# giesselmann/STRique

Hardware: AMD Instinct MI355X
Metric: reads/s for STRique 'count' on 50 kb r9.4 signals (higher is better)
Workload: dtype f32

## Files before the change

strique_amd/csrc/screen_kernels.h:

```cpp
#pragma once
#include <hip/hip_runtime.h>
#include <stdint.h>
#include "align_kernels.h"

#define STRQ_SCREEN_R 14
#define STRQ_SCREEN_S 6
#define STRQ_SCREEN_SEG 4
#define STRQ_SCREEN_CHUNK_COLS 128
#define STRQ_SCREEN_MAX_WINDOWS 4
#define STRQ_SCREEN2_CPL 5
#define STRQ_SCREEN2_LPF 29
#define STRQ_SCREEN2_LANE_B 32

namespace strq {

struct ScreenParams {
    int32_t sc;
    int32_t hh, v;
    int32_t cadd;
    int32_t slack;
    int32_t merge_gap;
    int32_t max_cand;
    int32_t margin;
};
// ... 4 lines not shown
    const int32_t* band_lo;
    int32_t* out;
    int32_t tsize;
    int32_t n, m, k, col_off;
    int32_t n_chunks;
    int32_t lane_last;
};

struct Screen2Task {
    const uint8_t* levels;
    const float* table[2];
    const int32_t* band_lo[2];
    int32_t* out[2];
    int32_t tsize[2], k[2];
    int32_t n, col_off, n_chunks;
};

struct ScreenWindows {
    int32_t n_win;
    int32_t lo[STRQ_SCREEN_MAX_WINDOWS], hi[STRQ_SCREEN_MAX_WINDOWS];
    float lower_bound;
    float upper_bound;
    int32_t n_cand;
};

int screen_plan(const AlignParams& p, int samples, int max_n, ScreenParams* sp);
static inline bool screen_flank_ok(int m) { return m >= 2 * STRQ_SCREEN_R && m <= 64 * STRQ_SCREEN_R; }
size_t screen_lds_bytes(int tsize);
int launch_screen(hipStream_t stream, const ScreenTask* tasks, int n_groups, int* queue, const ScreenParams& sp,
                  size_t lds_bytes, int tables_per_cu, int n_cu);
int screen2_plan(const AlignParams& p, int samples, int max_n, int merge, ScreenParams* sp);
static inline bool screen2_flank_ok(int m, int k) { return k >= 1 && k <= STRQ_SCREEN2_LPF * STRQ_SCREEN2_CPL && m == k * STRQ_SCREEN_S; }
size_t screen2_lds_bytes(int tsize_a, int tsize_b);
int launch_screen2(hipStream_t stream, const Screen2Task* tasks, int n_groups, int* queue, const ScreenParams& sp,
                   size_t lds_bytes, int groups_per_cu, int n_cu, int merge);
int launch_screen_windows(hipStream_t stream, const ScreenTask* tasks, int n_groups, const ScreenParams& sp,
                          const int32_t* bound_scaled, ScreenWindows* out, const int32_t* list = nullptr, const int32_t* theta_list = nullptr);

}
```

strique_amd/csrc/screen_kernels.hip:

```cpp
#include "strq_opt.h"
#include <hip/hip_runtime.h>
#include <stdint.h>
#include <stdlib.h>
#include <cmath>
#include "screen_kernels.h"

namespace strq {

namespace {

constexpr int R = STRQ_SCREEN_R, S = STRQ_SCREEN_S, SEG = STRQ_SCREEN_SEG;
constexpr int G = 2, C = 3;
static_assert(R == 14 && S == 6, "class expansion below is written for 14 rows per lane, 6 samples per class");

__device__ __forceinline__ int dpp_shr1(int v, int fill)
{
    return __builtin_amdgcn_update_dpp(fill, v, 0x138, 0xF, 0xF, false);
}
__device__ __forceinline__ int dpp_shr1_open(int v)
{
    return __builtin_amdgcn_mov_dpp(v, 0x138, 0xF, 0xF, true);
}
__device__ __forceinline__ int med3i(int a, int lo, int hi)
{
    int r;
    asm("v_med3_i32 %0, %1, %2, %3" : "=v"(r) : "v"(a), "v"(lo), "v"(hi));
    return r;
}
#define STRQ_SCREEN_BIAS 0x00800000
#ifndef STRQ_SCREEN_WPE
#define STRQ_SCREEN_WPE 6
#endif
__device__ __forceinline__ int max3i(int a, int b, int c)
{
    int r;
    asm("v_max3_f32 %0, %1, %2, %3" : "=v"(r) : "v"(a), "v"(b), "v"(c));
    return r;
}
// ... 239 lines not shown
            if (act) {
#pragma unroll
                for (int r = RPC * c; r < RPC * c + RPC; ++r) {
                    const int diagA = r == 0 ? upS : T[r - 1];
                    const int ta = max3i(diagA + scA[c], T[r], ta_prev);
                    if (r > 0) {
                        const int tb = max3i(ta_prev2 + scB[(r - 1) / RPC], ta_prev, tb_prev2);
                        T[r - 1] = tb; tb_prev2 = tb;
                    }
                    ta_prev2 = ta_prev; ta_prev = ta;
                }
                if (c == CPL - 1) {
                    const int tb = max3i(ta_prev2 + scB[c], ta_prev, tb_prev2);
                    T[R2 - 1] = tb;
                    SbotA = ta_prev;
                    upS = upB;
                    if constexpr (GROUPED) {
                        if (glast) { const int d = tb - gpot; gmax = d > gmax ? d : gmax; }
                    } else {
                        const int cA = ta_prev - potA + STRQ_SCREEN_BIAS, cB = okB ? tb - potBn + STRQ_SCREEN_BIAS : cA;
                        cmax = max3i(cmax, cA, cB);
                    }
                }
            }
            scA[c] = score(qa, c);
            if (c > 0) scB[c - 1] = score(qb, c - 1);
            if (c == CPL - 1) scB[c] = score(qb, c);
        }
        potB = potBn;
        qq = qn;
    }
};

__device__ __forceinline__ int load_chunk2(const Screen2Task& tk, int chunk, int lane)
{
    const int idx = (chunk * 64 + lane) * 2;
    int a = 0, b = 0;
    if (idx < tk.n) a = tk.levels[idx];
    if (idx + 1 < tk.n) b = tk.levels[idx + 1];
    return (a * 2) | ((b * 2) << 16);
}

template <int RPC, int CMG>
__device__ __forceinline__ void screen2_body(const Screen2Task* __restrict__ tasks, int n_groups, int* __restrict__ queue, const ScreenParams& sp)
{
    constexpr int R2 = RPC * CPL, MERGE = S / RPC;
    extern __shared__ uint32_t lds_all[];
    __shared__ int next_group;
    const int lane = threadIdx.x & 63, wave = threadIdx.x >> 6;
    const char* ldsb = reinterpret_cast<const char*>(lds_all);
    for (;;) {
        __syncthreads();
        if (threadIdx.x == 0) next_group = atomicAdd(queue, 1);
        __syncthreads();
        const int gi = __builtin_amdgcn_readfirstlane(next_group);
        if (gi >= n_groups) break;
        const Screen2Task& t0 = tasks[(size_t)gi * SEG];
        int base[2], zero_idx[2];
        base[0] = 0; zero_idx[0] = (t0.tsize[0] + 1) & ~1;
        base[1] = zero_idx[0] + 2; zero_idx[1] = base[1] + ((t0.tsize[1] + 1) & ~1);
        {
            uint16_t* dst = reinterpret_cast<uint16_t*>(lds_all);
            const float scf = (float)sp.sc;
#pragma unroll
            for (int f = 0; f < 2; ++f) {
                for (int i = threadIdx.x; i < t0.tsize[f]; i += 64 * SEG) dst[base[f] + i] = (uint16_t)(MERGE * ((int)ceilf(t0.table[f][i] * scf) + sp.cadd));
                if (threadIdx.x == 0) { dst[zero_idx[f]] = 0; dst[zero_idx[f] + 1] = 0; }
            }
        }
        __syncthreads();
        const Screen2Task& tk = tasks[(size_t)gi * SEG + wave];
        if (tk.n <= 0) continue;

        Lane2Const lc;
        const int f = lane >= LB ? 1 : 0, lf = lane - f * LB;
        {
#pragma unroll
            for (int c = 0; c < CPL; ++c) {
                const int k = lf * CPL + c;
                if (lf < LPF && k < tk.k[f]) {
                    const uint32_t d = (uint32_t)tk.band_lo[f][k];
                    const int lo = (int)(d & 255u), w1 = (int)((d >> 8) & 255u), off = (int)(d >> 16);
                    lc.lo2[c] = lo * 2; lc.hi2[c] = (lo + w1) * 2;
                    lc.off[c] = (base[f] + off - lo) * 2;
                } else {
                    lc.lo2[c] = 0; lc.hi2[c] = 0; lc.off[c] = zero_idx[f] * 2;
                }
            }
        }
        const uint64_t top_mask = 1ull | (1ull << LB);
        const int lMa = (tk.k[0] - 1) / CPL, lMb = LB + (tk.k[1] - 1) / CPL;
        Screen2<RPC, CMG> s2{ldsb, lc, top_mask, lane, tk.n, sp.hh};
        {
#pragma unroll
            for (int r = 0; r < R2; ++r) s2.T[r] = STRQ_SCREEN_BIAS;
            s2.SbotA = STRQ_SCREEN_BIAS; s2.upS = STRQ_SCREEN_BIAS;
            s2.potB = STRQ_SCREEN_BIAS - 2 * lane * sp.hh;
            s2.cmax = STRQ_SCREEN_BIAS; s2.gpot = 0; s2.gmax = 0;
        }
        const int nsteps = (tk.n + 1) / 2 + 63;
        int qcur = load_chunk2(tk, 0, lane);
        s2.prime(qcur);
        for (int t0s = 0; t0s < nsteps; t0s += 64) {
            const int qnext = load_chunk2(tk, t0s / 64 + 1, lane);
            const bool full = (t0s >= 63) && (2 * (t0s + 64) <= tk.n);
            const int send = nsteps - t0s < 64 ? nsteps - t0s : 64;
            if (full) {
                constexpr int U = CMG > 2 ? CMG : 2;
                s2.gmax = 0;
#pragma unroll 1
                for (int s = 0; s < 64 - U; s += U) {
#pragma unroll
                    for (int u = 0; u < U; ++u) s2.template step<false>(0, qcur, s + u + 1, u % CMG == 0, u % CMG == CMG - 1);
                }
#pragma unroll
                for (int u = 0; u < U - 1; ++u) s2.template step<false>(0, qcur, 64 - U + u + 1, u % CMG == 0, u % CMG == CMG - 1);
                s2.template step<false>(0, qnext, 0, CMG == 1, true);
                if constexpr (CMG > 1) s2.cmax = s2.gmax + STRQ_SCREEN_BIAS;
            } else {
                for (int s = 0; s < send; ++s) {
                    const int qsrc = s == 63 ? qnext : qcur, snext = (s + 1) & 63;
                    s2.template step<true>(t0s + s + 1, qsrc, snext);
                }
            }
            const int cma = __builtin_amdgcn_readlane(s2.cmax, lMa) - STRQ_SCREEN_BIAS;
            const int cmb = __builtin_amdgcn_readlane(s2.cmax, lMb) - STRQ_SCREEN_BIAS;
            if (lane == 0) { tk.out[0][t0s / 64] = cma; tk.out[1][t0s / 64] = cmb; }
            s2.cmax = STRQ_SCREEN_BIAS;
            qcur = qnext;
        }
    }
}

}

size_t screen2_lds_bytes(int tsize_a, int tsize_b)
{
    return (size_t)(((tsize_a + 1) & ~1) + 2 + ((tsize_b + 1) & ~1) + 2) * 2;
}

#ifndef STRQ_SCREEN3_CMG
#define STRQ_SCREEN3_CMG 2
#endif
#define STRQ_SCREEN2_ATTR(WPE_) __attribute__((amdgpu_flat_work_group_size(64 * STRQ_SCREEN_SEG, 64 * STRQ_SCREEN_SEG), amdgpu_waves_per_eu(WPE_, WPE_)))
__global__ void STRQ_SCREEN2_ATTR(6) align_screen3_kernel(const Screen2Task* __restrict__ tasks, int n_groups, int* __restrict__ queue, ScreenParams sp) { screen2_body<2, STRQ_SCREEN3_CMG>(tasks, n_groups, queue, sp); }
__global__ void STRQ_SCREEN2_ATTR(4) align_screen1_kernel(const Screen2Task* __restrict__ tasks, int n_groups, int* __restrict__ queue, ScreenParams sp) { screen2_body<6, 1>(tasks, n_groups, queue, sp); }

__global__ void __launch_bounds__(256)
screen_windows_kernel(const ScreenTask* __restrict__ tasks, int n_groups, ScreenParams sp,
                      const int32_t* __restrict__ bound_scaled, ScreenWindows* __restrict__ out,
                      const int32_t* __restrict__ list, const int32_t* __restrict__ theta_list)
{
    const int lane = threadIdx.x & 63;
    const int idx = blockIdx.x * (blockDim.x >> 6) + (threadIdx.x >> 6);
    if (idx >= n_groups) return;
    const int g = list ? list[idx] : idx;
    const ScreenTask* tg = tasks + (size_t)g * SEG;
    const int m = tg[0].m, lM = tg[0].lane_last;
    const int shift = -m * sp.v;
    int vmax = 0;
    for (int w = 0; w < SEG; ++w) {
        if (tg[w].n <= 0) continue;
        for (int c = lane; c < tg[w].n_chunks; c += 64) { const int v = tg[w].out[c]; vmax = v > vmax ? v : vmax; }
    }
#pragma unroll
    for (int d = 32; d >= 1; d >>= 1) { const int o = __shfl_xor(vmax, d, 64); vmax = o > vmax ? o : vmax; }
    ScreenWindows r;
    r.n_win = 0; r.n_cand = 0;
    for (int k = 0; k < STRQ_SCREEN_MAX_WINDOWS; ++k) { r.lo[k] = 0; r.hi[k] = 0; }
    const int drop = (sp.margin > 0 ? sp.margin : m) + 2 * sp.slack;
    int theta = theta_list ? theta_list[idx] : vmax - drop;
    if (!theta_list && sp.max_cand > 0) {
        auto count_at = [&](int t) {
            int n = 0;
            for (int w = 0; w < SEG; ++w) {
                if (tg[w].n <= 0) continue;
                for (int c = lane; c < tg[w].n_chunks; c += 64) n += tg[w].out[c] >= t;
            }
#pragma unroll
// ... 96 lines not shown
        if (hh < 1 || smax + v + hh > 65000.0) continue;
        const double top = 64.0 * R * (smax + v) + ((double)max_n + 256.0) * hh + smax + v + hh + (double)STRQ_SCREEN_BIAS;
        if (top > 2.0e9) continue;
        sp->sc = sc; sp->hh = (int)hh; sp->v = (int)v; sp->cadd = (int)(hh + v);
        {
            const double rows = 64.0 * R, maxval = rows * (double)p.dist_offset;
            double p2 = 1.0; while (p2 < maxval) p2 *= 2.0;
            const double adds = rows * (1.0 + (double)p.dist_offset / -(double)p.ext_h);
            const double e = adds * p2 / 16777216.0;
            if (!(e < 1.0e4)) continue;
            sp->slack = ((int)std::ceil(e) + 1) * sc;
        }
        sp->merge_gap = 3072; sp->margin = 0; sp->max_cand = 0;
        return 1;
    }
    return 0;
}

int screen2_plan(const AlignParams& p, int samples, int max_n, int merge, ScreenParams* sp)
{
    if (merge != 1 && merge != 3) return 0;
    if (!screen_plan(p, samples, max_n, sp)) return 0;
    while (sp->sc >= 16) {
        const double smax = std::ceil((double)p.dist_offset * sp->sc);
        if ((double)merge * (smax + sp->cadd) <= 65000.0) return 1;
        if ((sp->hh & 1) || (sp->v & 1)) return 0;
        sp->slack = (sp->slack / sp->sc) * (sp->sc / 2);
        sp->sc /= 2; sp->hh /= 2; sp->v /= 2; sp->cadd = sp->hh + sp->v;
    }
    return 0;
}

int launch_screen2(hipStream_t stream, const Screen2Task* tasks, int n_groups, int* queue, const ScreenParams& sp,
                   size_t lds_bytes, int groups_per_cu, int n_cu, int merge)
{
    if (n_groups <= 0) return 0;
    if (merge != 3 && merge != 1) return 2;
    auto kern = merge == 3 ? align_screen3_kernel : align_screen1_kernel;
    if (merge == 1 && groups_per_cu > 4) groups_per_cu = 4;
    if (groups_per_cu > 6) groups_per_cu = 6;
    (void)hipFuncSetAttribute((const void*)kern, hipFuncAttributeMaxDynamicSharedMemorySize, (int)lds_bytes);
    hipLaunchKernelGGL(kern, dim3(groups_per_cu * n_cu), dim3(64 * SEG), lds_bytes, stream, tasks, n_groups, queue, sp);
    return hipGetLastError() == hipSuccess ? 0 : 1;
}

int launch_screen(hipStream_t stream, const ScreenTask* tasks, int n_groups, int* queue, const ScreenParams& sp,
                  size_t lds_bytes, int tables_per_cu, int n_cu)
{
    if (n_groups <= 0) return 0;
    (void)hipFuncSetAttribute((const void*)align_screen_kernel, hipFuncAttributeMaxDynamicSharedMemorySize, (int)lds_bytes);
    hipLaunchKernelGGL(align_screen_kernel, dim3(tables_per_cu * n_cu), dim3(64 * SEG), lds_bytes, stream, tasks, n_groups, queue, sp);
    return hipGetLastError() == hipSuccess ? 0 : 1;
}

int launch_screen_windows(hipStream_t stream, const ScreenTask* tasks, int n_groups, const ScreenParams& sp,
                          const int32_t* bound_scaled, ScreenWindows* out, const int32_t* list, const int32_t* theta_list)
{
    if (n_groups <= 0) return 0;
    hipLaunchKernelGGL(screen_windows_kernel, dim3((n_groups + 3) / 4), dim3(256), 0, stream, tasks, n_groups, sp, bound_scaled, out, list, theta_list);
    return hipGetLastError() == hipSuccess ? 0 : 1;
}

}
```

strique_amd/csrc/strq_align_api.hip:

```cpp
#include <hip/hip_runtime.h>
#include <algorithm>
#include <cmath>
#include <climits>
#include <cstring>
#include <cstdlib>
#include <time.h>
#include <unistd.h>
#include <map>
#include <mutex>
#include <string>
#include <tuple>
#include <numeric>
#include <vector>
#include "../../include/strique_hip.h"
#include "strq_ctx.h"
#include "align_kernels.h"
#include "lut_kernels.h"
#include "align_generic.h"

using namespace strq;

#define STRQ_DBG(...) do { if (strq::opt("STRQ_DEBUG")) { fprintf(stderr, "[strq] " __VA_ARGS__); fprintf(stderr, "\n"); fflush(stderr); } } while (0)

namespace strq {
// ... 259 lines not shown
    if (hard_count > hard_cap) { c->err = "too many borderline table entries"; return STRQ_ERR_DEVICE; }
    bool any_rebuild = false;
    for (int j = 0; j < nj; ++j) any_rebuild |= info[j].n_hard < 0;
    auto level_vals_of = [&](int read, float* dst) -> int {
        STRQ_HIP(c, hipMemcpy(dst, b.d_level_val + (size_t)read * 256, 256 * 4, hipMemcpyDeviceToHost));
        return STRQ_OK;
    };
    if (hard_count > 0) {
        std::vector<HardEntry> he(hard_count); std::vector<float> hv(hard_count);
        STRQ_HIP(c, hipMemcpy(he.data(), d_hard, (size_t)hard_count * sizeof(HardEntry), hipMemcpyDeviceToHost));
        float lv[256]; int last_read = -1;
        for (int i = 0; i < hard_count; ++i) {
            const int rd = b.job_read[he[i].job];
            if (rd != last_read) { const int rc = level_vals_of(rd, lv); if (rc) return rc; last_read = rd; }
            hv[i] = host_cell_score(c->ap, lv[he[i].level], b.job_cls[he[i].job][he[i].k]);
        }
        STRQ_HIP(c, hipMemcpyAsync(d_hard_vals, hv.data(), (size_t)hard_count * 4, hipMemcpyHostToDevice, st));
        if (launch_lut_patch(st, d_jobs, d_hard, d_hard_vals, hard_count)) { c->err = "patch launch failed"; return STRQ_ERR_DEVICE; }
        STRQ_HIP(c, hipStreamSynchronize(st));
        if (b.handed) *b.handed = he;
    } else if (b.handed) b.handed->clear();
    if (any_rebuild) for (int j = 0; j < nj; ++j) if (info[j].n_hard < 0) {
        const int kk = jobs[j].k;
        std::vector<float> tab((size_t)kk * 256); std::vector<int32_t> blo(kk);
        float lv[256];
        { const int rc = level_vals_of(b.job_read[j], lv); if (rc) return rc; }
        for (int x = 0; x < kk; ++x) {
            float* row = &tab[(size_t)x * 256];
            for (int q = 0; q < 256; ++q) row[q] = host_cell_score(c->ap, lv[q], b.job_cls[j][x]);
            blo[x] = (int32_t)((255u << 8) | ((uint32_t)(x * 256) << 16));
        }
        STRQ_HIP(c, hipMemcpy(jobs[j].table, tab.data(), tab.size() * 4, hipMemcpyHostToDevice));
        STRQ_HIP(c, hipMemcpy(jobs[j].band_lo, blo.data(), (size_t)kk * 4, hipMemcpyHostToDevice));
        info[j].total = kk * 256;
    }
    b.hard_count = hard_count;
    return STRQ_OK;
}

static uint8_t* table3_slot(strq_ctx* c, size_t tab_off, int j)
{
    const size_t o = tab_off * 3 + (size_t)j * 8;
    return c->tables3.as<uint8_t>() + o - o % 4;
}

static int build_tables(CorePlan& p)
{
    strq_ctx* c = p.c; const AlignCoreIn& in = p.in;
    const int nb = p.nb, nj = p.nj;
    std::vector<LutJob>& jobs = p.jobs;
    jobs.resize(nj);
    TableBuild b;
    b.nj = nj; b.max_k = p.max_k; b.jobs = &jobs; b.d_level_val = in.d_level_val; b.after_tables = in.after_tables; b.info = &p.info;
    b.job_read.resize(nj); b.job_cls.resize(nj);
    for (int j = 0; j < nj; ++j) {
        const int i = p.job_align[j];
        jobs[j].level_val = in.d_level_val + (size_t)in.read[i] * 256;
        jobs[j].cls_val = c->flank_cls.as<float>() + p.cls_off[i] + p.job_k0[j];
        jobs[j].table = c->tables.as<float>() + p.tab_off[j];
        jobs[j].table3 = table3_slot(c, p.tab_off[j], j);
        jobs[j].band_lo = c->band_lo.as<int32_t>() + p.desc_off[j];
        jobs[j].k = p.job_k[j]; jobs[j].pad_ = 0;
        b.job_read[j] = in.read[i];
        b.job_cls[j] = &p.h_cls[p.cls_off[i] + p.job_k0[j]];
    }
    const int rc = run_table_build(c, p.st, b);
    if (rc) return rc;
    p.tab_total.assign(nb, 0);
    for (int j = 0; j < nj; ++j) p.tab_total[p.job_align[j]] = std::max(p.tab_total[p.job_align[j]], p.info[j].total);
    p.out.n_hard = b.hard_count;
    return STRQ_OK;
}

static void read_switches(CorePlan& p)
{
    const strq_ctx* c = p.c;
    p.collapsed = p.S == 6 && c->ap.open_h == c->ap.ext_h && c->ap.open_v == c->ap.ext_v;
    if (const char* e = strq::opt("STRQ_SEG")) { const int v = atoi(e); if (v >= 1 && v <= 4) p.seg_want = v; }
    if (const char* e = strq::opt("STRQ_TABLES")) { const int v = atoi(e); if (v >= 1 && v <= 8) p.max_tables = v; }
    if (const char* e = strq::opt("STRQ_MAX_WAVES")) { const int v = atoi(e); if (v >= 4 && v <= 16) p.max_waves = v; }
    p.allow_pack = p.collapsed && !strq::opt("STRQ_NO_PACK");
    if (const char* e = strq::opt("STRQ_OVERLAP")) { const int v = atoi(e); p.ov_cap = v > 0 ? v : (1 << 30); p.ov_fixed = true; }
    p.scr_forced = strq::opt("STRQ_SCREEN_ALWAYS") != nullptr;
    const char* mode_opt = strq::opt("STRQ_SCREEN_MODE");
    p.mode_fine = mode_opt && std::strcmp(mode_opt, "fine") == 0;
    p.mode_coarse = mode_opt && std::strcmp(mode_opt, "coarse") == 0;
}


struct ScreenJob {
    int flanks = 1;
    std::vector<int> al;
    std::vector<ScreenTask> views;
    std::vector<Screen2Task> t2;
    std::vector<int32_t> bound;
    std::vector<size_t> out_off;
    size_t out_words = 0, lds_bytes = 0;
    double steps = 0;
};

struct ScreenRules {
    int merge;
    int groups_per_cu;
    const char* lds_err;
    bool below_bound_free;
    bool count_untaken;
    bool judge;
    double max_cols;
    int* pause; int* fail;
};

static void screen_tasks(CorePlan& p, const ScreenParams& sp, ScreenJob& j)
{
    constexpr int SSEG = STRQ_SCREEN_SEG;
    const AlignCoreIn& in = p.in;
    const int F = j.flanks, ng = (int)j.al.size() / F;
    if (F == 2) j.t2.resize((size_t)ng * SSEG);
    j.views.resize(j.al.size() * SSEG);
    j.bound.resize(j.al.size());
    j.out_off.assign(j.al.size() * SSEG, 0);
    for (int g = 0; g < ng; ++g) {
        const int* a = &j.al[(size_t)g * F];
        const int n = in.n[a[0]];
        const int m_big = F == 2 ? std::max(in.m[a[0]], in.m[a[1]]) : in.m[a[0]];
        const int ov_worst = align_segment_overlap(p.c->ap, m_big), ov_s = overlap_for(p, m_big, ov_worst, 16);
        Piece pc[SSEG];
        const int used = cut(n, SSEG, ov_s, pc);
        j.lds_bytes = std::max(j.lds_bytes, F == 2 ? screen2_lds_bytes(p.info[p.J0[a[0]]].total, p.info[p.J0[a[1]]].total) : screen_lds_bytes(p.info[p.J0[a[0]]].total));
        for (int f = 0; f < F; ++f)
            j.bound[(size_t)g * F + f] = used <= 1 ? INT32_MIN / 2 : (ov_s >= ov_worst ? 0 : (int32_t)std::ceil((double)align_segment_min_score(p.c->ap, in.m[a[f]], ov_s) * sp.sc));
        for (int w = 0; w < SSEG; ++w) {
            Screen2Task t; std::memset(&t, 0, sizeof(t));
            t.levels = in.d_levels + in.read_off[in.read[a[0]]] + pc[w].col_off;
            t.n = pc[w].n; t.col_off = pc[w].col_off;
            t.n_chunks = pc[w].n > 0 ? (align_num_steps(pc[w].n) + 63) / 64 : 0;
            for (int f = 0; f < F; ++f) {
                const LutJob& job = p.jobs[p.J0[a[f]]];
                t.table[f] = job.table; t.band_lo[f] = job.band_lo; t.tsize[f] = p.info[p.J0[a[f]]].total; t.k[f] = in.k[a[f]];
                ScreenTask v; std::memset(&v, 0, sizeof(v));
                v.n = pc[w].n; v.m = in.m[a[f]]; v.k = in.k[a[f]]; v.col_off = pc[w].col_off; v.n_chunks = t.n_chunks;
                if (F == 2) v.lane_last = f * STRQ_SCREEN2_LANE_B + (in.k[a[f]] - 1) / STRQ_SCREEN2_CPL;
                else { v.levels = t.levels; v.table = t.table[0]; v.band_lo = t.band_lo[0]; v.tsize = t.tsize[0]; v.lane_last = (v.m - 1) / STRQ_SCREEN_R; }
                j.out_off[((size_t)g * F + f) * SSEG + w] = j.out_words; j.out_words += (size_t)t.n_chunks;
                j.views[((size_t)g * F + f) * SSEG + w] = v;
            }
            if (pc[w].n > 0) j.steps += align_num_steps(pc[w].n);
            if (F == 2) j.t2[(size_t)g * SSEG + w] = t;
        }
    }
}

static int run_screen(CorePlan& p, ScreenJob& j, const ScreenParams& sp, const ScreenRules& r)
{
    constexpr int SSEG = STRQ_SCREEN_SEG;
    strq_ctx* c = p.c; const AlignCoreIn& in = p.in;
    hipStream_t st = p.st;
    const int nv = (int)j.al.size();
    if (j.lds_bytes > 160 * 1024 - 64) { c->err = r.lds_err; return STRQ_ERR_UNSUPPORTED; }
    const int groups = std::max(1, std::min(r.groups_per_cu, (int)((160 * 1024 - 64) / j.lds_bytes)));
    auto aligned = [](size_t bytes) { return (bytes + 255) & ~(size_t)255; };
    const size_t t2_bytes = aligned(j.t2.size() * sizeof(Screen2Task)), task_bytes = aligned(j.views.size() * sizeof(ScreenTask));
    const size_t bound_bytes = aligned((size_t)nv * 4), win_bytes = aligned((size_t)nv * sizeof(ScreenWindows));
    STRQ_HIP(c, c->screen.reserve(t2_bytes + task_bytes + bound_bytes + win_bytes + j.out_words * 4 + 256));
    char* base = c->screen.as<char>();
    Screen2Task* d_t2 = reinterpret_cast<Screen2Task*>(base);
    ScreenTask* d_st = reinterpret_cast<ScreenTask*>(base + t2_bytes);
    int32_t* d_bound = reinterpret_cast<int32_t*>(base + t2_bytes + task_bytes);
    ScreenWindows* d_win = reinterpret_cast<ScreenWindows*>(base + t2_bytes + task_bytes + bound_bytes);
    int32_t* d_out = reinterpret_cast<int32_t*>(base + t2_bytes + task_bytes + bound_bytes + win_bytes);
    for (size_t x = 0; x < j.views.size(); ++x) j.views[x].out = d_out + j.out_off[x];
    if (j.flanks == 2)
        for (int v = 0; v < nv; ++v) for (int w = 0; w < SSEG; ++w) j.t2[(size_t)(v / 2) * SSEG + w].out[v % 2] = j.views[(size_t)v * SSEG + w].out;
    if (j.flanks == 2) STRQ_HIP(c, hipMemcpyAsync(d_t2, j.t2.data(), j.t2.size() * sizeof(Screen2Task), hipMemcpyHostToDevice, st));
    STRQ_HIP(c, hipMemcpyAsync(d_st, j.views.data(), j.views.size() * sizeof(ScreenTask), hipMemcpyHostToDevice, st));
    STRQ_HIP(c, hipMemcpyAsync(d_bound, j.bound.data(), (size_t)nv * 4, hipMemcpyHostToDevice, st));
    STRQ_HIP(c, hipEventRecord(c->ev[5], st));
    int* queue = c->queue.as<int>() + STRQ_QUEUE_FIRST - 1;
    if (j.flanks == 2) {
        if (launch_screen2(st, d_t2, nv / 2, queue, sp, j.lds_bytes, groups, c->n_cu, r.merge)) { c->err = "coarse screen launch failed"; return STRQ_ERR_DEVICE; }
    } else {
        if (launch_screen(st, d_st, nv, queue, sp, j.lds_bytes, groups, c->n_cu)) { c->err = "screen launch failed"; return STRQ_ERR_DEVICE; }
    }
    STRQ_HIP(c, hipEventRecord(c->ev[6], st));
    if (launch_screen_windows(st, d_st, nv, sp, d_bound, d_win)) { c->err = "screen windows launch failed"; return STRQ_ERR_DEVICE; }
    std::vector<ScreenWindows> hw((size_t)nv);
    STRQ_HIP(c, hipMemcpyAsync(hw.data(), d_win, hw.size() * sizeof(ScreenWindows), hipMemcpyDeviceToHost, st));
    STRQ_HIP(c, hipStreamSynchronize(st));
    c->screen_ran = true; c->screen_mode_last = r.merge > 1 ? 2 : 1; c->coarse_merge_last = r.merge;
    if (const char* path = strq::opt("STRQ_SCREEN_DUMP")) {
        std::vector<int32_t> ho(j.out_words);
        STRQ_HIP(c, hipMemcpy(ho.data(), d_out, j.out_words * 4, hipMemcpyDeviceToHost));
        if (FILE* fp = fopen(path, "wb")) {
            const int32_t hdr[8] = {nv, sp.sc, sp.hh, sp.v, j.flanks, SSEG, sp.slack, r.merge};
            fwrite(hdr, 4, 8, fp);
            for (int v = 0; v < nv; ++v) {
                const int32_t gh[4] = {j.al[v], j.al[v], j.bound[v], j.views[(size_t)v * SSEG].lane_last};
                fwrite(gh, 4, 4, fp);
                for (int w = 0; w < SSEG; ++w) {
                    const ScreenTask& t = j.views[(size_t)v * SSEG + w];
                    const int32_t th[4] = {t.col_off, t.n, t.m, t.n_chunks};
                    fwrite(th, 4, 4, fp);
                    fwrite(ho.data() + (t.out - d_out), 4, (size_t)t.n_chunks, fp);
                }
                fwrite(&hw[(size_t)v], sizeof(ScreenWindows), 1, fp);
            }
            fclose(fp);
        }
    }
    if (const char* e = strq::opt("STRQ_SCREEN_TEST_RAISE")) {
        const float up = (float)atof(e);
        for (auto& w : hw) w.lower_bound += up;
    }
    int windowed = 0, heavy = 0, below_bound = 0; double cols = 0, all = 0;
    for (int v = 0; v < nv; ++v) {
        const int al = j.al[v];
        const ScreenWindows& w = hw[(size_t)v];
        c->screen_stats[1] += 1; c->screen_stats[7] += w.n_cand;
        double mine = in.n[al];
        if (w.n_win > 0) {
            p.wins[al] = w; c->screen_stats[2] += 1; ++windowed; mine = 0;
            for (int k = 0; k < w.n_win; ++k) { c->screen_stats[4] += w.hi[k] - w.lo[k] + 1; mine += w.hi[k] - w.lo[k] + 1 + 4096; }
// ... 926 lines not shown
        info_out[5 * j + 3] = reported[j].n_hard; info_out[5 * j + 4] = info[j].total;
    }
    STRQ_HIP(c, hipMemcpy(band_lo, c->band_lo.p, cls_tot * 4, hipMemcpyDeviceToHost));
    STRQ_HIP(c, hipMemcpy(table, c->tables.p, tab_tot * 4, hipMemcpyDeviceToHost));
    for (int j = 0; j < n_jobs; ++j)
        STRQ_HIP(c, hipMemcpy(planes + (size_t)cls_off[j] * 768 + (size_t)j * 8, jobs[j].table3, (size_t)jobs[j].k * 768 + 8, hipMemcpyDeviceToHost));
    *n_handed = (int32_t)he.size();
    for (size_t i = 0; i < he.size() && (int64_t)i < handed_cap; ++i) {
        handed[4 * i] = he[i].job; handed[4 * i + 1] = he[i].k; handed[4 * i + 2] = he[i].level; handed[4 * i + 3] = he[i].index;
    }
    return STRQ_OK;
}

int strq_last_overlap(const strq_ctx* c, double out[4])
{
    if (!c || !out) return STRQ_ERR_ARG;
    for (int i = 0; i < 4; ++i) out[i] = c->overlap[i];
    return STRQ_OK;
}
int strq_last_screen(const strq_ctx* c, double out[8])
{
    if (!c || !out) return STRQ_ERR_ARG;
    for (int i = 0; i < 8; ++i) out[i] = c->screen_stats[i];
    return STRQ_OK;
}

int strq_last_screen_mode(const strq_ctx* c, int32_t out[8])
{
    if (!c || !out) return STRQ_ERR_ARG;
    for (int i = 0; i < 8; ++i) out[i] = 0;
    out[0] = c->screen_mode_last; out[1] = c->coarse_pause; out[2] = c->screen_pause; out[3] = (int32_t)c->coarse_margin;
    out[5] = (int32_t)std::min<int64_t>(c->look2_served, INT32_MAX);
    out[4] = c->screen_mode_last ? c->coarse_merge_last : 0;
    return STRQ_OK;
}

int strq_last_second_round(const strq_ctx* c, int64_t out[2])
{
    if (!c || !out) return STRQ_ERR_ARG;
    out[0] = c->second_round[0]; out[1] = c->second_round[1];
    return STRQ_OK;
}

int strq_last_viterbi_launches(const strq_ctx* c, int32_t out[4])
{
    if (!c || !out) return STRQ_ERR_ARG;
    std::memcpy(out, c->vit_launches, sizeof(c->vit_launches));
    return STRQ_OK;
}

int strq_last_geometry(const strq_ctx* c, int32_t out[8])
{
    if (!c || !out) return STRQ_ERR_ARG;
    std::memcpy(out, c->geometry, sizeof(c->geometry));
    return STRQ_OK;
}

int strq_align_batch(strq_ctx* c, int64_t n_align, int64_t n_reads, const uint8_t* levels,
                     const int64_t* read_off, const float* level_val, const int32_t* align_read,
                     const float* flank, const int64_t* flank_off, int32_t samples,
                     float* score, int64_t* j_end, int64_t* j0, int32_t* rec)
{
    strq::CtxScope scope_(c);
    if (!c) return STRQ_ERR_ARG;
    if (n_align < 0 || n_reads < 0 || (n_align > 0 && (!levels || !read_off || !level_val || !align_read || !flank || !flank_off)) || samples < 1) {
        c->err = "bad argument"; return STRQ_ERR_ARG;
// ... 160 lines not shown
```

strique_amd/csrc/strq_ctx.h:

```cpp
#pragma once
#include <hip/hip_runtime.h>
#include <stdint.h>
#include <string>
#include <vector>
#include <map>
#include <cstdio>
#include <functional>
#include <mutex>
#include <atomic>
#include <utility>
#include "align_kernels.h"
#include "viterbi_kernels.h"
#include "forward_kernels.h"
#include "mod_llr_kernels.h"
#include "variant_kernels.h"
#include "screen_kernels.h"
#include "strq_opt.h"

namespace strq {

inline std::atomic<int64_t> live_allocations[2];

template <bool PINNED> struct OwnedBuf {
    void* p = nullptr;
// ... 71 lines not shown
    int32_t var_mode = -1, var_nb = 0;
};

}

struct strq_ctx {
    std::map<std::string, std::string> options;
    mutable std::mutex options_mu;
    int device = 0;
    int n_cu = 0;
    hipStream_t stream = nullptr;
    hipStream_t side_stream = nullptr;
    hipEvent_t ev_fork = nullptr, side_join = nullptr;
    hipEvent_t ev[8] = {};
    strq::AlignParams ap{-2.0f, -8.0f, -2.0f, -8.0f, 8.0f, -16.0f};
    std::string err;
    float timing[8] = {};
    double counters[8] = {};
    int32_t geometry[8] = {};
    int32_t vit_launches[4] = {};
    int64_t second_round[2] = {};
    strq::DevBuf redo_total;
    int64_t look2_served = 0;
    double screen_stats[8] = {};
    double overlap[4] = {};
    bool screen_ran = false;
    int screen_pause = 0;
    int coarse_pause = 0;
    int coarse_fail = 0, screen_fail = 0;
    float coarse_margin = 384.0f;
    float aborted_fwd_ms = 0, aborted_screen_ms = 0;
    int screen_mode_last = 0;
    int coarse_merge_last = 0;
    
    strq::DevBuf levels, level_val, flank_cls, tables, tables3, band_lo, col0, ckpt, rec, tasks, results,
        queue, scratch, lutinfo, hard, misc, vit_x, vit_tasks, vit_bp, vit_path, bnd,
        gen_codes, gen_table, gen_bnd, gen_trace, gen_hard,
        screen,
        ckpt2;
    std::vector<strq::HostModel*> models;
    void* detect = nullptr;
    size_t max_ws_bytes = (size_t)96 << 30;
    std::vector<float> score_fracs; double mean_n = 0;
};

namespace strq {
struct CtxScope { const strq_ctx* prev; explicit CtxScope(const strq_ctx* c); ~CtxScope(); };
int align_core(strq_ctx* c, const AlignCoreIn& in, AlignCoreOut& out);
int align_core_times(strq_ctx* c, float* t_lut, float* t_fwd, float* t_tr);
int align_validate_flank(strq_ctx* c, const float* f, int64_t m, int samples, int* k_out, int* R_out, int* NS_out);
size_t align_workspace_bytes(int n, int m, int R, int NS);
float host_cell_score(const AlignParams& p, float h, float v);
void detect_state_free(strq_ctx* c);
int detect_drain(strq_ctx* c);
int viterbi_launch_status(int vrc);
int forward_model(strq_ctx* c, HostModel* hm);
void host_stats_batch(const double* signals, const int64_t* offsets, int64_t n_reads, bool want_raw, double* out,
                      const double* const* reads = nullptr);
}

#define STRQ_ENTER(ctx)                                                                        \
    if (!(ctx)) return STRQ_ERR_ARG;                                                           \
    strq::CtxScope scope_(ctx);                                                                \
    STRQ_HIP(ctx, hipSetDevice((ctx)->device))

#define STRQ_HIP(ctx, call)                                                                    \
// ... 17 lines not shown
```

strique_amd/ffi.py:

```python
import ctypes
import os

import numpy as np

_HERE = os.path.dirname(os.path.abspath(__file__))
LIB_PATH = os.environ.get("STRQ_LIB") or os.path.join(_HERE, "lib", "libstrique_hip.so")

STRQ_OK, STRQ_ERR_ARG, STRQ_ERR_DEVICE, STRQ_ERR_UNSUPPORTED, STRQ_ERR_NOMEM = 0, 1, 2, 3, 4

SCAN_SYMBOLS = ("strq_scan_batch_reads", "strq_scan_set", "strq_scan_clear", "strq_batch_fetch_scan")

_lib = None


class StriqueHipError(RuntimeError):
    def __init__(self, code, message):
        RuntimeError.__init__(self, "libstrique_hip error %d: %s" % (code, message))
        self.code = code


def _torch_hip_runtime():
    import importlib.util
    try:
        spec = importlib.util.find_spec("torch")
# ... 196 lines not shown
                                               ctypes.c_int32(samples), _ptr(score), _ptr(j_end), _ptr(j0), _ptr(rec)))
        return score, j_end, j0, rec

    def last_timing(self):
        t = np.zeros(8, np.float32)
        self._check(self._lib.strq_last_timing(self._h, _ptr(t)))
        return t

    def last_counters(self):
        t = np.zeros(8, np.float64)
        self._check(self._lib.strq_last_counters(self._h, _ptr(t)))
        return t

    def last_viterbi_launches(self):
        g = np.zeros(4, np.int32)
        self._check(self._lib.strq_last_viterbi_launches(self._h, _ptr(g)))
        return dict(zip(("launches", "register_resident", "lane_layout", "general"), (int(v) for v in g)))

    def last_second_round(self):
        g = np.zeros(2, np.int64)
        self._check(self._lib.strq_last_second_round(self._h, _ptr(g)))
        return int(g[0]), int(g[1])

    def last_screen(self):
        g = np.zeros(8, np.float64)
        self._check(self._lib.strq_last_screen(self._h, _ptr(g)))
        keys = ("ms", "screened", "windowed", "whole_read", "window_columns", "wave_steps", "scale", "candidate_chunks")
        out = dict(zip(keys, (float(v) for v in g)))
        m = np.zeros(8, np.int32)
        self._check(self._lib.strq_last_screen_mode(self._h, _ptr(m)))
        out["mode"] = {0: None, 1: "fine", 2: "coarse"}.get(int(m[0]))
        out["coarse_pause"], out["fine_pause"], out["coarse_margin"], out["merge"] = int(m[1]), int(m[2]), int(m[3]), int(m[4])
        out["second_look"] = int(m[5])
        return out

    def last_overlap(self):
        g = np.zeros(4, np.float64)
        self._check(self._lib.strq_last_overlap(self._h, _ptr(g)))
        return dict(zip(("viterbi_ms", "under_screen_ms", "under_alignment_stage_ms", "sub_batches"), (float(v) for v in g)))

    def last_geometry(self):
        g = np.zeros(8, np.int32)
        self._check(self._lib.strq_last_geometry(self._h, _ptr(g)))
        keys = ("waves_per_alignment", "tables_per_cu", "wpe", "rows_per_lane", "packed", "overlap_first", "overlap_worst", "launch_groups")
        return dict(zip(keys, (int(v) for v in g)))

    def model_create(self, baked):
        mid = ctypes.c_int32(-1)
        arrs = [_c(baked.in_ptr, np.int32), _c(baked.in_src, np.int32), _c(baked.in_logp, np.float64),
                _c(baked.emis_kind, np.int32), _c(baked.emis_a, np.float64), _c(baked.emis_b, np.float64),
                _c(baked.emis_c, np.float64), _c(baked.count_inc, np.int32), _c(baked.tag, np.int32)]
        hints = getattr(baked, 'hint_slot', None) is not None and (np.asarray(baked.hint_slot)[:baked.silent_start] >= 0).all()
        arrs += [_c(baked.hint_slot, np.int32) if hints else None, _c(baked.hint_lane, np.int32) if hints else None]
        self._check(self._lib.strq_model_create(self._h, ctypes.c_int32(baked.n_states), ctypes.c_int32(baked.silent_start),
                                                ctypes.c_int32(baked.start), ctypes.c_int32(baked.end),
                                                *[_ptr(a) for a in arrs], ctypes.byref(mid)))
        psum = getattr(baked, 'in_logp_sum', None)
        if psum is not None and len(psum) == len(baked.in_logp) and np.all(psum >= baked.in_logp) and not np.array_equal(psum, baked.in_logp):
            self._check(self._lib.strq_model_set_forward_logp(self._h, mid, _ptr(_c(baked.in_logp_sum, np.float64))))
        self.last_positions_rc = self.last_positions_error = None
        if getattr(baked, 'pos_kind', None) is not None:
            rc = self._lib.strq_model_set_positions(self._h, mid, _ptr(_c(baked.pos_kind, np.int32)), _ptr(_c(baked.pos_index, np.int32)))
            self.last_positions_rc = rc
            self.last_positions_error = self._lib.strq_last_error(self._h).decode() if rc == STRQ_ERR_UNSUPPORTED else None
            if rc not in (STRQ_OK, STRQ_ERR_UNSUPPORTED):
                self._check(rc)
# ... 398 lines not shown
```

Measured before the change: 24340.

## Lay out coarse screen score tables per lane in LDS to avoid bank conflicts

Adds a lane-striped LDS layout for the two-flank coarse screen. Each lane's five classes are stacked as 128-byte rows with a per-lane 2-byte slot, so table lookups across a wave land in distinct banks instead of colliding in one shared flat table. The level pairs are pre-shifted by the row size so the address clamp works directly in bytes. The change adds per-lane table filling work and a fixed LDS footprint of rows times 128 bytes, which may reduce occupancy. The old flat layout stays available through STRQ_SCREEN_LDS=rows.

```diff
diff --git a/strique_amd/csrc/screen_kernels.h b/strique_amd/csrc/screen_kernels.h
--- a/strique_amd/csrc/screen_kernels.h
+++ b/strique_amd/csrc/screen_kernels.h
@@ -60,8 +60,11 @@
 int screen2_plan(const AlignParams& p, int samples, int max_n, int merge, ScreenParams* sp);
 static inline bool screen2_flank_ok(int m, int k) { return k >= 1 && k <= STRQ_SCREEN2_LPF * STRQ_SCREEN2_CPL && m == k * STRQ_SCREEN_S; }
 size_t screen2_lds_bytes(int tsize_a, int tsize_b);
+int screen2_lanes_rows(int need_a, int need_b);
+bool screen2_lanes_fit(int rows);
+size_t screen2_lanes_lds_bytes(int rows);
 int launch_screen2(hipStream_t stream, const Screen2Task* tasks, int n_groups, int* queue, const ScreenParams& sp,
-                   size_t lds_bytes, int groups_per_cu, int n_cu, int merge);
+                   size_t lds_bytes, int groups_per_cu, int n_cu, int merge, int lanes_rows);
 int launch_screen_windows(hipStream_t stream, const ScreenTask* tasks, int n_groups, const ScreenParams& sp,
                           const int32_t* bound_scaled, ScreenWindows* out, const int32_t* list = nullptr, const int32_t* theta_list = nullptr);
 
diff --git a/strique_amd/csrc/screen_kernels.hip b/strique_amd/csrc/screen_kernels.hip
--- a/strique_amd/csrc/screen_kernels.hip
+++ b/strique_amd/csrc/screen_kernels.hip
@@ -4,6 +4,7 @@
 #include <stdlib.h>
 #include <cmath>
 #include "screen_kernels.h"
+#include "screen_lds_layout.h"
 
 namespace strq {
 
@@ -309,23 +310,27 @@
     }
 };
 
+template <int SHIFT>
 __device__ __forceinline__ int load_chunk2(const Screen2Task& tk, int chunk, int lane)
 {
     const int idx = (chunk * 64 + lane) * 2;
     int a = 0, b = 0;
     if (idx < tk.n) a = tk.levels[idx];
     if (idx + 1 < tk.n) b = tk.levels[idx + 1];
-    return (a * 2) | ((b * 2) << 16);
-}
-
-template <int RPC, int CMG>
-__device__ __forceinline__ void screen2_body(const Screen2Task* __restrict__ tasks, int n_groups, int* __restrict__ queue, const ScreenParams& sp)
+    return (a << SHIFT) | (b << (SHIFT + 16));
+}
+
+template <int RPC, int CMG, bool LANES>
+__device__ __forceinline__ void screen2_body(const Screen2Task* __restrict__ tasks, int n_groups, int* __restrict__ queue, const ScreenParams& sp, int lds_rows)
 {
     constexpr int R2 = RPC * CPL, MERGE = S / RPC;
+    constexpr int QSHIFT = LANES ? screen_lanes::ROW_SHIFT : 1;
+    static_assert(CPL == screen_lanes::CPL, "screen_lds_layout.h stacks the lane's five classes");
     extern __shared__ uint32_t lds_all[];
     __shared__ int next_group;
     const int lane = threadIdx.x & 63, wave = threadIdx.x >> 6;
     const char* ldsb = reinterpret_cast<const char*>(lds_all);
+    const int f = lane >= LB ? 1 : 0, lf = lane - f * LB;
     for (;;) {
         __syncthreads();
         if (threadIdx.x == 0) next_group = atomicAdd(queue, 1);
@@ -333,25 +338,50 @@
         const int gi = __builtin_amdgcn_readfirstlane(next_group);
         if (gi >= n_groups) break;
         const Screen2Task& t0 = tasks[(size_t)gi * SEG];
-        int base[2], zero_idx[2];
+        const float scf = (float)sp.sc;
+        Lane2Const lc;
+        if constexpr (LANES) {
+            uint32_t desc[CPL];
+            int nc = 0, rowbase[CPL];
+#pragma unroll
+            for (int c = 0; c < CPL; ++c) {
+                const int k = lf * CPL + c;
+                const bool in = lf < LPF && k < t0.k[f];
+                desc[c] = in ? (uint32_t)t0.band_lo[f][k] : 0u;
+                nc += in ? 1 : 0;
+            }
+            screen_lanes::row_bases(desc, nc, rowbase);
+            char* dst = reinterpret_cast<char*>(lds_all);
+            if (wave == 0) *reinterpret_cast<uint16_t*>(dst + screen_lanes::slot(lane)) = 0;
+#pragma unroll
+            for (int c = 0; c < CPL; ++c) {
+                const screen_lanes::ClassAddr a = c < nc ? screen_lanes::class_addr(lane, rowbase[c], desc[c]) : screen_lanes::padding_addr(lane);
+                lc.lo2[c] = a.lo2; lc.hi2[c] = a.hi2; lc.off[c] = a.off;
+                if (c < nc) {
+                    const float* src = t0.table[f] + screen_lanes::desc_off(desc[c]);
+                    const int w1 = screen_lanes::desc_w1(desc[c]);
+                    for (int i = (wave - rowbase[c]) & (SEG - 1); i <= w1; i += SEG)
+                        if (rowbase[c] + i < lds_rows)
+                            *reinterpret_cast<uint16_t*>(dst + screen_lanes::entry_address(lane, rowbase[c], i)) = (uint16_t)(MERGE * ((int)ceilf(src[i] * scf) + sp.cadd));
+                }
+            }
+        }
+        [[maybe_unused]] int base[2], zero_idx[2];
         base[0] = 0; zero_idx[0] = (t0.tsize[0] + 1) & ~1;
         base[1] = zero_idx[0] + 2; zero_idx[1] = base[1] + ((t0.tsize[1] + 1) & ~1);
-        {
+        if constexpr (!LANES) {
             uint16_t* dst = reinterpret_cast<uint16_t*>(lds_all);
-            const float scf = (float)sp.sc;
-#pragma unroll
-            for (int f = 0; f < 2; ++f) {
-                for (int i = threadIdx.x; i < t0.tsize[f]; i += 64 * SEG) dst[base[f] + i] = (uint16_t)(MERGE * ((int)ceilf(t0.table[f][i] * scf) + sp.cadd));
-                if (threadIdx.x == 0) { dst[zero_idx[f]] = 0; dst[zero_idx[f] + 1] = 0; }
+#pragma unroll
+            for (int ff = 0; ff < 2; ++ff) {
+                for (int i = threadIdx.x; i < t0.tsize[ff]; i += 64 * SEG) dst[base[ff] + i] = (uint16_t)(MERGE * ((int)ceilf(t0.table[ff][i] * scf) + sp.cadd));
+                if (threadIdx.x == 0) { dst[zero_idx[ff]] = 0; dst[zero_idx[ff] + 1] = 0; }
             }
         }
         __syncthreads();
         const Screen2Task& tk = tasks[(size_t)gi * SEG + wave];
         if (tk.n <= 0) continue;
 
-        Lane2Const lc;
-        const int f = lane >= LB ? 1 : 0, lf = lane - f * LB;
-        {
+        if constexpr (!LANES) {
 #pragma unroll
             for (int c = 0; c < CPL; ++c) {
                 const int k = lf * CPL + c;
@@ -376,10 +406,10 @@
             s2.cmax = STRQ_SCREEN_BIAS; s2.gpot = 0; s2.gmax = 0;
         }
         const int nsteps = (tk.n + 1) / 2 + 63;
-        int qcur = load_chunk2(tk, 0, lane);
+        int qcur = load_chunk2<QSHIFT>(tk, 0, lane);
         s2.prime(qcur);
         for (int t0s = 0; t0s < nsteps; t0s += 64) {
-            const int qnext = load_chunk2(tk, t0s / 64 + 1, lane);
+            const int qnext = load_chunk2<QSHIFT>(tk, t0s / 64 + 1, lane);
             const bool full = (t0s >= 63) && (2 * (t0s + 64) <= tk.n);
             const int send = nsteps - t0s < 64 ? nsteps - t0s : 64;
             if (full) {
@@ -416,12 +446,20 @@
     return (size_t)(((tsize_a + 1) & ~1) + 2 + ((tsize_b + 1) & ~1) + 2) * 2;
 }
 
+int screen2_lanes_rows(int need_a, int need_b) { return screen_lanes::rows_bound(need_a, need_b); }
+bool screen2_lanes_fit(int rows) { return screen_lanes::fits(rows); }
+size_t screen2_lanes_lds_bytes(int rows) { return screen_lanes::bytes(rows); }
+
 #ifndef STRQ_SCREEN3_CMG
 #define STRQ_SCREEN3_CMG 2
 #endif
 #define STRQ_SCREEN2_ATTR(WPE_) __attribute__((amdgpu_flat_work_group_size(64 * STRQ_SCREEN_SEG, 64 * STRQ_SCREEN_SEG), amdgpu_waves_per_eu(WPE_, WPE_)))
-__global__ void STRQ_SCREEN2_ATTR(6) align_screen3_kernel(const Screen2Task* __restrict__ tasks, int n_groups, int* __restrict__ queue, ScreenParams sp) { screen2_body<2, STRQ_SCREEN3_CMG>(tasks, n_groups, queue, sp); }
-__global__ void STRQ_SCREEN2_ATTR(4) align_screen1_kernel(const Screen2Task* __restrict__ tasks, int n_groups, int* __restrict__ queue, ScreenParams sp) { screen2_body<6, 1>(tasks, n_groups, queue, sp); }
+#define STRQ_SCREEN2_ARGS const Screen2Task* __restrict__ tasks, int n_groups, int* __restrict__ queue, ScreenParams sp, int lds_rows
+__global__ void STRQ_SCREEN2_ATTR(6) align_screen3_kernel(STRQ_SCREEN2_ARGS) { screen2_body<2, STRQ_SCREEN3_CMG, true>(tasks, n_groups, queue, sp, lds_rows); }
+__global__ void STRQ_SCREEN2_ATTR(4) align_screen1_kernel(STRQ_SCREEN2_ARGS) { screen2_body<6, 1, true>(tasks, n_groups, queue, sp, lds_rows); }
+__global__ void STRQ_SCREEN2_ATTR(6) align_screen3_rows_kernel(STRQ_SCREEN2_ARGS) { screen2_body<2, STRQ_SCREEN3_CMG, false>(tasks, n_groups, queue, sp, lds_rows); }
+__global__ void STRQ_SCREEN2_ATTR(4) align_screen1_rows_kernel(STRQ_SCREEN2_ARGS) { screen2_body<6, 1, false>(tasks, n_groups, queue, sp, lds_rows); }
+#undef STRQ_SCREEN2_ARGS
 
 __global__ void __launch_bounds__(256)
 screen_windows_kernel(const ScreenTask* __restrict__ tasks, int n_groups, ScreenParams sp,
@@ -584,15 +622,17 @@
 }
 
 int launch_screen2(hipStream_t stream, const Screen2Task* tasks, int n_groups, int* queue, const ScreenParams& sp,
-                   size_t lds_bytes, int groups_per_cu, int n_cu, int merge)
+                   size_t lds_bytes, int groups_per_cu, int n_cu, int merge, int lanes_rows)
 {
     if (n_groups <= 0) return 0;
     if (merge != 3 && merge != 1) return 2;
-    auto kern = merge == 3 ? align_screen3_kernel : align_screen1_kernel;
+    const bool lanes = lanes_rows > 0;
+    if (lanes && (!screen_lanes::fits(lanes_rows) || lds_bytes < screen_lanes::bytes(lanes_rows))) return 2;
+    auto kern = merge == 3 ? (lanes ? align_screen3_kernel : align_screen3_rows_kernel) : (lanes ? align_screen1_kernel : align_screen1_rows_kernel);
     if (merge == 1 && groups_per_cu > 4) groups_per_cu = 4;
     if (groups_per_cu > 6) groups_per_cu = 6;
     (void)hipFuncSetAttribute((const void*)kern, hipFuncAttributeMaxDynamicSharedMemorySize, (int)lds_bytes);
-    hipLaunchKernelGGL(kern, dim3(groups_per_cu * n_cu), dim3(64 * SEG), lds_bytes, stream, tasks, n_groups, queue, sp);
+    hipLaunchKernelGGL(kern, dim3(groups_per_cu * n_cu), dim3(64 * SEG), lds_bytes, stream, tasks, n_groups, queue, sp, lanes_rows);
     return hipGetLastError() == hipSuccess ? 0 : 1;
 }
 
diff --git a/strique_amd/csrc/screen_lds_layout.h b/strique_amd/csrc/screen_lds_layout.h
--- /dev/null
+++ b/strique_amd/csrc/screen_lds_layout.h
@@ -0,0 +1,60 @@
+#pragma once
+#include <stddef.h>
+#include <stdint.h>
+
+#if defined(__HIPCC__) || defined(__CUDACC__)
+#define STRQ_LAYOUT_HD __host__ __device__ __forceinline__
+#else
+#define STRQ_LAYOUT_HD inline
+#endif
+
+namespace strq {
+namespace screen_lanes {
+
+constexpr int ROW_BYTES = 128;
+constexpr int ROW_SHIFT = 7;
+constexpr int CPL = 5;
+static_assert(ROW_BYTES == 1 << ROW_SHIFT && 255 * ROW_BYTES < 65536, "a scaled level has to fit the 16-bit half of the level pair");
+
+constexpr int MAX_ROWS = 264;
+constexpr size_t MAX_BYTES = (size_t)MAX_ROWS * ROW_BYTES;
+
+STRQ_LAYOUT_HD int desc_lo(uint32_t d) { return (int)(d & 255u); }
+STRQ_LAYOUT_HD int desc_w1(uint32_t d) { return (int)((d >> 8) & 255u); }
+STRQ_LAYOUT_HD int desc_off(uint32_t d) { return (int)(d >> 16); }
+
+STRQ_LAYOUT_HD int slot(int lane) { return (lane & 31) * 4 + (lane >> 5) * 2; }
+
+STRQ_LAYOUT_HD int row_bases(const uint32_t* desc, int n, int (&rowbase)[CPL])
+{
+    int rows = 1;
+    for (int c = 0; c < CPL; ++c) {
+        if (c < n) { rowbase[c] = rows; rows += desc_w1(desc[c]) + 1; }
+        else rowbase[c] = 0;
+    }
+    return rows;
+}
+
+struct ClassAddr { int lo2, hi2, off; };
+STRQ_LAYOUT_HD ClassAddr class_addr(int lane, int rowbase, uint32_t desc)
+{
+    const int lo = desc_lo(desc), w1 = desc_w1(desc);
+    return ClassAddr{lo * ROW_BYTES, (lo + w1) * ROW_BYTES, slot(lane) + (rowbase - lo) * ROW_BYTES};
+}
+STRQ_LAYOUT_HD ClassAddr padding_addr(int lane) { return ClassAddr{0, 0, slot(lane)}; }
+
+STRQ_LAYOUT_HD int address(const ClassAddr& a, int level)
+{
+    const int q = level * ROW_BYTES;
+    const int m = q < a.lo2 ? a.lo2 : (q > a.hi2 ? a.hi2 : q);
+    return m + a.off;
+}
+STRQ_LAYOUT_HD int entry_address(int lane, int rowbase, int i) { return slot(lane) + (rowbase + i) * ROW_BYTES; }
+
+STRQ_LAYOUT_HD size_t bytes(int rows) { return (size_t)rows * ROW_BYTES; }
+
+STRQ_LAYOUT_HD int rows_bound(int need_a, int need_b) { return 1 + CPL * (need_a > need_b ? need_a : need_b); }
+STRQ_LAYOUT_HD bool fits(int rows) { return rows <= MAX_ROWS; }
+
+}
+}
diff --git a/strique_amd/csrc/strq_align_api.hip b/strique_amd/csrc/strq_align_api.hip
--- a/strique_amd/csrc/strq_align_api.hip
+++ b/strique_amd/csrc/strq_align_api.hip
@@ -315,7 +315,7 @@
         }
         STRQ_HIP(c, hipMemcpy(jobs[j].table, tab.data(), tab.size() * 4, hipMemcpyHostToDevice));
         STRQ_HIP(c, hipMemcpy(jobs[j].band_lo, blo.data(), (size_t)kk * 4, hipMemcpyHostToDevice));
-        info[j].total = kk * 256;
+        info[j].total = kk * 256; info[j].need = 256;
     }
     b.hard_count = hard_count;
     return STRQ_OK;
@@ -379,6 +379,7 @@
     std::vector<int32_t> bound;
     std::vector<size_t> out_off;
     size_t out_words = 0, lds_bytes = 0;
+    int lanes_rows = 0;
     double steps = 0;
 };
 
@@ -410,6 +411,7 @@
         Piece pc[SSEG];
         const int used = cut(n, SSEG, ov_s, pc);
         j.lds_bytes = std::max(j.lds_bytes, F == 2 ? screen2_lds_bytes(p.info[p.J0[a[0]]].total, p.info[p.J0[a[1]]].total) : screen_lds_bytes(p.info[p.J0[a[0]]].total));
+        if (F == 2) j.lanes_rows = std::max(j.lanes_rows, screen2_lanes_rows(p.info[p.J0[a[0]]].need, p.info[p.J0[a[1]]].need));
         for (int f = 0; f < F; ++f)
             j.bound[(size_t)g * F + f] = used <= 1 ? INT32_MIN / 2 : (ov_s >= ov_worst ? 0 : (int32_t)std::ceil((double)align_segment_min_score(p.c->ap, in.m[a[f]], ov_s) * sp.sc));
         for (int w = 0; w < SSEG; ++w) {
@@ -439,6 +441,11 @@
     strq_ctx* c = p.c; const AlignCoreIn& in = p.in;
     hipStream_t st = p.st;
     const int nv = (int)j.al.size();
+    int lanes_rows = 0;
+    if (j.flanks == 2) {
+        const char* e = strq::opt("STRQ_SCREEN_LDS");
+        if (!(e && std::strcmp(e, "rows") == 0) && screen2_lanes_fit(j.lanes_rows)) { lanes_rows = j.lanes_rows; j.lds_bytes = screen2_lanes_lds_bytes(lanes_rows); }
+    }
     if (j.lds_bytes > 160 * 1024 - 64) { c->err = r.lds_err; return STRQ_ERR_UNSUPPORTED; }
     const int groups = std::max(1, std::min(r.groups_per_cu, (int)((160 * 1024 - 64) / j.lds_bytes)));
     auto aligned = [](size_t bytes) { return (bytes + 255) & ~(size_t)255; };
@@ -460,7 +467,7 @@
     STRQ_HIP(c, hipEventRecord(c->ev[5], st));
     int* queue = c->queue.as<int>() + STRQ_QUEUE_FIRST - 1;
     if (j.flanks == 2) {
-        if (launch_screen2(st, d_t2, nv / 2, queue, sp, j.lds_bytes, groups, c->n_cu, r.merge)) { c->err = "coarse screen launch failed"; return STRQ_ERR_DEVICE; }
+        if (launch_screen2(st, d_t2, nv / 2, queue, sp, j.lds_bytes, groups, c->n_cu, r.merge, lanes_rows)) { c->err = "coarse screen launch failed"; return STRQ_ERR_DEVICE; }
     } else {
         if (launch_screen(st, d_st, nv, queue, sp, j.lds_bytes, groups, c->n_cu)) { c->err = "screen launch failed"; return STRQ_ERR_DEVICE; }
     }
@@ -470,6 +477,7 @@
     STRQ_HIP(c, hipMemcpyAsync(hw.data(), d_win, hw.size() * sizeof(ScreenWindows), hipMemcpyDeviceToHost, st));
     STRQ_HIP(c, hipStreamSynchronize(st));
     c->screen_ran = true; c->screen_mode_last = r.merge > 1 ? 2 : 1; c->coarse_merge_last = r.merge;
+    c->screen_lds_last = j.flanks == 2 ? (lanes_rows > 0 ? 1 : 2) : 0;
     if (const char* path = strq::opt("STRQ_SCREEN_DUMP")) {
         std::vector<int32_t> ho(j.out_words);
         STRQ_HIP(c, hipMemcpy(ho.data(), d_out, j.out_words * 4, hipMemcpyDeviceToHost));
@@ -1462,6 +1470,7 @@
     out[0] = c->screen_mode_last; out[1] = c->coarse_pause; out[2] = c->screen_pause; out[3] = (int32_t)c->coarse_margin;
     out[5] = (int32_t)std::min<int64_t>(c->look2_served, INT32_MAX);
     out[4] = c->screen_mode_last ? c->coarse_merge_last : 0;
+    out[6] = c->screen_mode_last ? c->screen_lds_last : 0;
     return STRQ_OK;
 }
 
diff --git a/strique_amd/csrc/strq_ctx.h b/strique_amd/csrc/strq_ctx.h
--- a/strique_amd/csrc/strq_ctx.h
+++ b/strique_amd/csrc/strq_ctx.h
@@ -127,6 +127,7 @@
     float aborted_fwd_ms = 0, aborted_screen_ms = 0;
     int screen_mode_last = 0;
     int coarse_merge_last = 0;
+    int screen_lds_last = 0;
     
     strq::DevBuf levels, level_val, flank_cls, tables, tables3, band_lo, col0, ckpt, rec, tasks, results,
         queue, scratch, lutinfo, hard, misc, vit_x, vit_tasks, vit_bp, vit_path, bnd,
diff --git a/strique_amd/ffi.py b/strique_amd/ffi.py
--- a/strique_amd/ffi.py
+++ b/strique_amd/ffi.py
@@ -252,6 +252,7 @@
         out["mode"] = {0: None, 1: "fine", 2: "coarse"}.get(int(m[0]))
         out["coarse_pause"], out["fine_pause"], out["coarse_margin"], out["merge"] = int(m[1]), int(m[2]), int(m[3]), int(m[4])
         out["second_look"] = int(m[5])
+        out["lds_layout"] = {0: None, 1: "lanes", 2: "rows"}.get(int(m[6]))
         return out
 
     def last_overlap(self):
```

Measured after the change: 25000, median of 6. 1.03x the previous value.
